# oooolga/Ctrl-V

Hardware: AMD Instinct MI355X
Metric: denoising steps/sec, SVD+ControlNet 25f 576x1024 (higher is better)
Workload: dtype bf16; 1 GPU; box2video: ControlNet + UNet forward, CFG batch 2, 25 frames, latent 72x128, 25-step Karras Euler schedule, random-init SVD-XT weights; clips_per_gpu=1, parallelism=clip-shard x1, hip_graph=True

## Files before the change

### ctrlv_amd/csrc/abi.hip

```cpp
#include <stdarg.h>
#include <stdlib.h>

#include <mutex>

#include "common.h"

#ifndef CTRLV_BUILD_ID
#define CTRLV_BUILD_ID "unstamped"
#endif

static thread_local char g_err[512] = "";
void ctrlv_set_error(const char* fmt, ...) {
  va_list ap;
  va_start(ap, fmt);
  vsnprintf(g_err, sizeof(g_err), fmt, ap);
  va_end(ap);
}

const ctrlv_debug_t& ctrlv_debug() {
  static const ctrlv_debug_t dbg = [] {
    auto env = [](const char* name, int dflt) { const char* e = getenv(name); return e ? atoi(e) : dflt; };
    ctrlv_debug_t d;
    d.w16 = env("CTRLV_W16", 1);
    d.splitk = env("CTRLV_SPLITK", 1);
    d.force_tile = env("CTRLV_GEMM_FORCE_TILE", 0);
    d.conv_halo = env("CTRLV_CONV_HALO", 1);
    d.gn_fused = env("CTRLV_GN_FUSED", 1);
    d.gn_cross = env("CTRLV_GN_CROSS", 1);
    d.gn_rev = env("CTRLV_GN_REV", 1);
    d.gn_rows = env("CTRLV_GN_ROWS", 256);
    if (d.gn_rows < 32 || d.gn_rows > 1024) d.gn_rows = 256;
    d.ln_rows = env("CTRLV_LN_ROWS", 1);
    d.ff_fused = env("CTRLV_FF_FUSED", 1);
    d.ff_ln = env("CTRLV_FF_LN", 0);
    d.pp_balanced = env("CTRLV_PP_BALANCED", 1);
    d.pp_cgrp = env("CTRLV_PP_CGRP", 0);
    d.attn_rows = env("CTRLV_ATTN_ROWS", 0);
    d.temporal_fused = env("CTRLV_TEMPORAL_FUSED", 1);
    d.wgrad_pp = env("CTRLV_WGRAD_PP", 1);
    d.wgrad_slabs = env("CTRLV_WGRAD_SLABS", 0);
    d.up_phase = env("CTRLV_UP_PHASE", 1);
    return d;
  }();
  return dbg;
}

int ctrlv_current_device() {
  int dev = 0;
  if (hipGetDevice(&dev) != hipSuccess || dev < 0 || dev >= CTRLV_MAX_DEVICES) dev = 0;
  return dev;
}

int ctrlv_num_cu(int dev) {
  static int cu[CTRLV_MAX_DEVICES] = {};
  static std::mutex mu;
  std::lock_guard<std::mutex> lk(mu);
  if (cu[dev] == 0) {
    int n = 0;
    if (hipDeviceGetAttribute(&n, hipDeviceAttributeMultiprocessorCount, dev) != hipSuccess || n <= 0) n = 256;
    cu[dev] = n;
  }
  return cu[dev];
}

extern "C" int ctrlv_last_error(char* buf, size_t n) {
  if (buf && n) {
    strncpy(buf, g_err, n - 1);
    buf[n - 1] = 0;
  }
  return (int)strlen(g_err);
}

extern "C" int ctrlv_abi_version(void) { return 22; }
static_assert(sizeof(ctrlv_gemm_desc) == 264 && offsetof(ctrlv_gemm_desc, ld_raw) == 192 && offsetof(ctrlv_gemm_desc, pad_br) == 196 &&
                  offsetof(ctrlv_gemm_desc, raw_out) == 200,
              "ctrlv_gemm_desc layout changed: that is an ABI bump");
extern "C" int ctrlv_elem_dtype(void) { return CTRLV_ELEM_DTYPE; }

extern "C" int ctrlv_build_id(char* buf, size_t n) {
  static const char marker[] = "CTRLV_BUILD_ID=" CTRLV_BUILD_ID;
  const char* id = marker + 15;
  if (buf && n) {
    strncpy(buf, id, n - 1);
    buf[n - 1] = 0;
  }
  return (int)strlen(id);
}
// ... 1 lines not shown
```

### ctrlv_amd/csrc/ff_fused.hip

```cpp
#include <type_traits>

#include "common.h"
#include "gemm_pp_kernel.h"

namespace {

constexpr int kC = 320, kHid = 1280, kChunks = kHid / 16;
constexpr int kTileM = 128;
#ifndef CTRLV_FF_GEA
#define CTRLV_FF_GEA 6
#endif
constexpr int kGeA = CTRLV_FF_GEA;
constexpr int kNQ = 6;
constexpr int kW1Pieces = 21;
constexpr int kW1Slot = kW1Pieces * 1024, kW2Slot = 10 * 1024;
constexpr int kStgOff = 0;
constexpr int kHfOff = kStgOff + 8 * 4096;
constexpr int kW1Off = kHfOff + 16 * 1024;
constexpr int kW2Off = kW1Off + 3 * kW1Slot;
constexpr int kTabOff = kW2Off + 4 * kW2Slot;
constexpr int kSmem = kTabOff + kGeluTabBytes;
static_assert(kSmem <= 160 * 1024, "fused feed-forward tile does not fit the LDS");

struct FfArgs {
  const el_t* x; int ldx;
  const el_t* w1f; const el_t* w2f;
  ctrlv_gemm_desc o;
  const float* vtab; int vdiv, vmod, ldv;
  const float* ln_g; const float* ln_b; float ln_eps;
  const float* lnv; int ln_vdiv, ln_vmod, ln_ldv;
};

template <int EPI, bool LO = false, bool LN = false>
__global__ __launch_bounds__(512) void ff_fused_kernel(const FfArgs a) {
#if defined(__HIP_DEVICE_COMPILE__)
  extern __shared__ __attribute__((aligned(1024))) char smem[];
  const int lane = threadIdx.x & 63;
  const int wid = __builtin_amdgcn_readfirstlane(threadIdx.x >> 6);
  const int rg = wid & 3, hh = wid >> 2;
  const int r32 = lane & 31, hsel = lane >> 5;
  const ctrlv_gemm_desc& d = a.o;
  const int M = d.M;
  const int tiles = (M + kTileM - 1) / kTileM, G = gridDim.x;

  CTRLV_CLOCK_BEGIN();
  gelu_table_fill(smem + kTabOff, threadIdx.x, 512);

  const __amdgpu_buffer_rsrc_t rsW1 = __builtin_amdgcn_make_buffer_rsrc((void*)a.w1f, 0, kChunks * kW1Slot, 0x00020000);
  const __amdgpu_buffer_rsrc_t rsW2 = __builtin_amdgcn_make_buffer_rsrc((void*)a.w2f, 0, kChunks * kW2Slot, 0x00020000);
  const __amdgpu_buffer_rsrc_t rsX = __builtin_amdgcn_make_buffer_rsrc((void*)a.x, 0, (int)((long)d.M * a.ldx * 2), 0x00020000);
  const __amdgpu_buffer_rsrc_t rsB2 = __builtin_amdgcn_make_buffer_rsrc((void*)(d.bias ? d.bias : (const float*)a.w1f), 0,
                                                                         d.bias ? kC * 4 : 0, 0x00020000);
  auto dma_w1 = [&](int chunk, int g) {
    char* s1 = smem + kW1Off + (g % 3) * kW1Slot;
#pragma unroll
    for (int k = 0; k < 6; ++k) {
      const int pi = k * 4 + rg;
      if (pi < kW1Pieces)
        __builtin_amdgcn_raw_ptr_buffer_load_lds(rsW1, LDS_PTR(s1 + pi * 1024), 16, lane * 16, chunk * kW1Slot + pi * 1024, 0, 0);
    }
  };
  auto dma_w2 = [&](int chunk, int g) {
    char* s2 = smem + kW2Off + (g & 3) * kW2Slot;
#pragma unroll
    for (int k = 0; k < 3; ++k) {
      const int pi = k * 4 + rg;
      if (pi < 10)
        __builtin_amdgcn_raw_ptr_buffer_load_lds(rsW2, LDS_PTR(s2 + pi * 1024), 16, lane * 16, chunk * kW2Slot + pi * 1024, 0, 0);
    }
  };
  for (int i = threadIdx.x * 16; i < 4 * kW2Slot; i += 512 * 16) *(uint4*)(smem + kW2Off + i) = make_uint4(0, 0, 0, 0);
  if (hh == 0) dma_w1(0, 0); else dma_w1(1, 1);
  wait_vmcnt<0>();
  __syncthreads();
  const char* tab = smem + kTabOff;
  const unsigned tab_lds = (unsigned)(unsigned long)LDS_PTR(smem + kTabOff);
  char* const hfx = smem + kHfOff + rg * 4096 + lane * 16;
  const unsigned xone1 = hsel == 0 ? (CTRLV_ELEM_DTYPE == 1 ? 0x3C003C00u : 0x3F803F80u) : 0u;

  int gbase = 0;
  elx8 xr[20];
  u32x4_t ini_b, ini_v;
  const __amdgpu_buffer_rsrc_t rsVt = __builtin_amdgcn_make_buffer_rsrc(
      (void*)(a.vtab ? a.vtab : (const float*)a.w1f), 0, a.vtab ? (int)((long)a.vmod * a.ldv * 4) : 0, 0x00020000);
  auto tile_loads = [&](int tile) {
    const int bm = tile * kTileM;
    const unsigned xoff = (unsigned)(bm + rg * 32 + r32) * (unsigned)(a.ldx * 2) + 16 * hsel;
#pragma unroll
    for (int ks = 0; ks < 20; ++ks)
      xr[ks] = __builtin_bit_cast(elx8, __builtin_amdgcn_raw_buffer_load_b128(rsX, xoff, ks * 32, 0));
    const unsigned col4 = lane < 40 ? (unsigned)(hh * 160 + lane * 4) * 4 : 0xFFFFFFFFu;
    ini_b = __builtin_amdgcn_raw_buffer_load_b128(rsB2, col4, 0, 0);
    ini_v = __builtin_amdgcn_raw_buffer_load_b128(rsVt, col4, a.vtab ? ((bm / a.vdiv) % a.vmod) * (a.ldv * 4) : 0, 0);
  };
  tile_loads(blockIdx.x);
  for (int tile = blockIdx.x; tile < tiles; tile += G, gbase += kChunks) {
    const int bm = tile * kTileM;
    const int m = bm + rg * 32 + r32;
#ifdef CTRLV_FF_STAMP
    unsigned long long st_tb; asm volatile("s_memtime %0\n\ts_waitcnt lgkmcnt(0)" : "=s"(st_tb)::"memory");
#endif
    if constexpr (LN) {
      const float* lv = a.lnv ? a.lnv + (long)((m / a.ln_vdiv) % a.ln_vmod) * a.ln_ldv + 8 * hsel : nullptr;
      auto raw8 = [&](int ks, float* f) {
        unpack_elx8(__builtin_bit_cast(uint4, xr[ks]), f);
        if (lv) {
          const float4 p = *(const float4*)(lv + ks * 16), q = *(const float4*)(lv + ks * 16 + 4);
          f[0] += p.x; f[1] += p.y; f[2] += p.z; f[3] += p.w; f[4] += q.x; f[5] += q.y; f[6] += q.z; f[7] += q.w;
        }
      };
      float pilot;
      {
        float f0[8];
        raw8(0, f0);
        pilot = __shfl(f0[0], r32);
      }
      float sm = 0.f, sq = 0.f;
#pragma unroll
      for (int ks = 0; ks < 20; ++ks) {
        float f[8];
        raw8(ks, f);
#pragma unroll
        for (int e = 0; e < 8; ++e) { const float dl = f[e] - pilot; sm += dl; sq += dl * dl; }
        if (ks % 5 == 4) __builtin_amdgcn_sched_barrier(0);
      }
      sm += __shfl_xor(sm, 32);
      sq += __shfl_xor(sq, 32);
      const float dm = sm * (1.0f / kC);
      const float var = sq * (1.0f / kC) - dm * dm;
      const float mean = pilot + dm, rstd = rsqrtf((var > 0.f ? var : 0.f) + a.ln_eps);
      const float* gp = a.ln_g + 8 * hsel;
      const float* bp = a.ln_b + 8 * hsel;
#pragma unroll
      for (int ks = 0; ks < 20; ++ks) {
        float f[8];
        raw8(ks, f);
        const float4 g0 = *(const float4*)(gp + ks * 16), g1 = *(const float4*)(gp + ks * 16 + 4);
        const float4 b0 = *(const float4*)(bp + ks * 16), b1v = *(const float4*)(bp + ks * 16 + 4);
        const float gg[8] = {g0.x, g0.y, g0.z, g0.w, g1.x, g1.y, g1.z, g1.w};
        const float bb[8] = {b0.x, b0.y, b0.z, b0.w, b1v.x, b1v.y, b1v.z, b1v.w};
#pragma unroll
        for (int e = 0; e < 8; ++e) f[e] = (f[e] - mean) * rstd * gg[e] + bb[e];
        uint4 o = pack_elx8(f);
        if (!(m < M)) o = make_uint4(0, 0, 0, 0);
        xr[ks] = __builtin_bit_cast(elx8, o);
        if (ks % 5 == 4) __builtin_amdgcn_sched_barrier(0);
      }
    }
    f32x16 acc[1][5];
    char* const stg = smem + kStgOff + wid * 4096;
    {
      const f32x4 b = __builtin_bit_cast(f32x4, ini_b), w = __builtin_bit_cast(f32x4, ini_v);
      if (lane < 40) *(float4*)(stg + lane * 16) = make_float4(b.x + w.x, b.y + w.y, b.z + w.z, b.w + w.w);
      __builtin_amdgcn_wave_barrier();
#pragma unroll
      for (int i = 0; i < 20; ++i) {
        const int n = i >> 2, q = i & 3;
        const float4 v = *(const float4*)(stg + (n * 32 + 8 * q + 4 * hsel) * 4);
        acc[0][n][4 * q] = v.x; acc[0][n][4 * q + 1] = v.y; acc[0][n][4 * q + 2] = v.z; acc[0][n][4 * q + 3] = v.w;
      }
      asm volatile("s_waitcnt lgkmcnt(0)" ::: "memory");
    }
#ifdef CTRLV_FF_STAMP
#define FSTAMP(v) unsigned long long v; asm volatile("s_memtime %0\n\ts_waitcnt lgkmcnt(0)" : "=s"(v)::"memory")
    unsigned long long st_g1 = 0, st_ge = 0, st_b = 0, st_bar = 0, st_dma = 0, st_tile0;
    { FSTAMP(tt0); st_tile0 = tt0; }
#else
#define FSTAMP(v)
#endif
    elx8 hcur, hprev;
    {
      const uint4 z = make_uint4(0, 0, 0, 0);
      hcur = hprev = __builtin_bit_cast(elx8, z);
    }
    auto geglu_part = [&](auto e0c, auto e1c, const float* av, const float* gv, float* h) {
      constexpr int E0 = decltype(e0c)::value, E1 = decltype(e1c)::value, NE = E1 - E0;
      float fr[NE ? NE : 1];
      f32x2_t te[NE ? NE : 1];
#pragma unroll
      for (int e = 0; e < NE; ++e) {
#pragma clang fp contract(off)
        float tq = __builtin_fmaf(gv[E0 + e], 100.0f, 512.0f);
        tq = __builtin_amdgcn_fmed3f(tq, 0.0f, 1023.99994f);
        fr[e] = __builtin_amdgcn_fractf(tq);
        const unsigned addr = tab_lds + (unsigned)((int)tq) * 8u;
        asm volatile("ds_read_b64 %0, %1" : "=v"(te[e]) : "v"(addr));
      }
      static_assert(NE == 0 || NE == 2 || NE == 4 || NE == 6 || NE == 8, "columns per part");
      if constexpr (NE == 8)
        asm volatile("s_waitcnt lgkmcnt(0)"
                     : "+v"(te[0]), "+v"(te[1]), "+v"(te[2]), "+v"(te[3]), "+v"(te[4]), "+v"(te[5]), "+v"(te[6]), "+v"(te[7]));
      if constexpr (NE == 2) asm volatile("s_waitcnt lgkmcnt(0)" : "+v"(te[0]), "+v"(te[1]));
      if constexpr (NE == 4) asm volatile("s_waitcnt lgkmcnt(0)" : "+v"(te[0]), "+v"(te[1]), "+v"(te[2]), "+v"(te[3]));
      if constexpr (NE == 6)
        asm volatile("s_waitcnt lgkmcnt(0)" : "+v"(te[0]), "+v"(te[1]), "+v"(te[2]), "+v"(te[3]), "+v"(te[4]), "+v"(te[5]));
#pragma unroll
      for (int e = 0; e < NE; ++e) h[E0 + e] = geglu_tab_finish(av[E0 + e], gv[E0 + e], fr[e], make_float2(te[e].x, te[e].y));
    };
    uint32_t hpk[kGeA / 2];
    float ak[kGeA < 8 ? 8 - kGeA : 1], gk[kGeA < 8 ? 8 - kGeA : 1];
    auto seg_g1 = [&](int t) {
      FSTAMP(t0);
      __builtin_amdgcn_s_setprio(2);
      const char* s1 = smem + kW1Off + ((gbase + t) % 3) * kW1Slot + lane * 16;
      elx8 wq[kNQ];
#pragma unroll
      for (int i = 0; i < kNQ; ++i) wq[i] = *(const elx8*)(s1 + i * 1024);
      f32x16 a1;
#pragma unroll
      for (int e = 0; e < 16; ++e) a1[e] = 0.f;
      __builtin_amdgcn_sched_barrier(0);
#pragma unroll
      for (int ks = 0; ks < 21; ++ks) {
        elx8 xf;
        if (ks == 20) {
          unsigned one = xone1;
          asm volatile("" : "+v"(one));
          xf = __builtin_bit_cast(elx8, make_uint4(one, 0, 0, 0));
        } else {
          xf = xr[ks];
        }
        a1 = mfma_32x32x16(wq[ks % kNQ], xf, a1);
        if (ks + kNQ < 21) wq[ks % kNQ] = *(const elx8*)(s1 + (ks + kNQ) * 1024);
        __builtin_amdgcn_sched_barrier(0);
      }
      FSTAMP(t1);
      float av[8], gv[8], h[8];
#pragma unroll
      for (int e = 0; e < 8; ++e) { av[e] = a1[e]; gv[e] = a1[8 + e]; }
      geglu_part(std::integral_constant<int, 0>{}, std::integral_constant<int, kGeA>{}, av, gv, h);
#pragma unroll
      for (int e = 0; e < kGeA / 2; ++e) hpk[e] = pack_elx2(h[2 * e], h[2 * e + 1]);
#pragma unroll
      for (int e = 0; e < 8 - kGeA; ++e) { ak[e] = av[kGeA + e]; gk[e] = gv[kGeA + e]; }
      __builtin_amdgcn_s_setprio(0);
#ifdef CTRLV_FF_STAMP
      FSTAMP(t2);
      st_g1 += t1 - t0; st_ge += t2 - t1;
#endif
    };
    auto seg_ge = [&](int t) {
      FSTAMP(t1b);
      float av[8], gv[8], h[8];
#pragma unroll
      for (int e = 0; e < 8 - kGeA; ++e) { av[kGeA + e] = ak[e]; gv[kGeA + e] = gk[e]; }
      geglu_part(std::integral_constant<int, kGeA>{}, std::integral_constant<int, 8>{}, av, gv, h);
      uint32_t hw[4];
#pragma unroll
      for (int e = 0; e < 4; ++e) hw[e] = e < kGeA / 2 ? hpk[e] : pack_elx2(h[2 * e], h[2 * e + 1]);
      const uint4 hp = make_uint4(hw[0], hw[1], hw[2], hw[3]);
      *(uint4*)(hfx + (t & 3) * 1024) = hp;
      hprev = hcur;
      hcur = __builtin_bit_cast(elx8, hp);
#ifdef CTRLV_FF_STAMP
      FSTAMP(t2);
      st_ge += t2 - t1b;
#endif
    };
    auto seg_dma = [&](int t) {
      FSTAMP(t0);
      dma_w1((t + 2) % kChunks, gbase + t + 2);
      if ((t & 1) == 0) { dma_w2(t, gbase + t); dma_w2(t + 1, gbase + t + 1); }
#ifdef CTRLV_FF_STAMP
      FSTAMP(t1);
      st_dma += t1 - t0;
#endif
    };
    auto seg_b = [&](int j) {
      FSTAMP(t0);
      const int c0 = 2 * j;
      const bool live = j >= 0 && j < kChunks / 2;
      const elx8 hpart = *(const elx8*)(hfx + ((c0 + (hh ^ 1)) & 3) * 1024);
      const char* s2a = smem + kW2Off + ((gbase + c0) & 3) * kW2Slot + (5 * hh) * 1024 + lane * 16;
      const char* s2b = smem + kW2Off + ((gbase + c0 + 1) & 3) * kW2Slot + (5 * hh) * 1024 + lane * 16;
      elx8 vq[6];
#pragma unroll
      for (int i = 0; i < 6; ++i) vq[i] = *(const elx8*)((i < 5 ? s2a + i * 1024 : s2b + (i - 5) * 1024));
      const uint4 hz = make_uint4(0, 0, 0, 0);
      const uint4 hp_u = __builtin_bit_cast(uint4, hpart);
      const uint4 own_u = hh == 0 ? __builtin_bit_cast(uint4, hprev) : __builtin_bit_cast(uint4, hcur);
      const uint4 h0_u = !live ? hz : hh == 0 ? own_u : hp_u;
      const uint4 h1_u = !live ? hz : hh == 0 ? hp_u : own_u;
      const elx8 h0 = __builtin_bit_cast(elx8, h0_u), h1 = __builtin_bit_cast(elx8, h1_u);
      __builtin_amdgcn_sched_barrier(0);
#pragma unroll
      for (int i = 0; i < 10; ++i) {
        acc[0][i % 5] = mfma_32x32x16(vq[i % 6], i < 5 ? h0 : h1, acc[0][i % 5]);
        if (i + 6 < 10) vq[i % 6] = *(const elx8*)(s2b + (i + 6 - 5) * 1024);
        __builtin_amdgcn_sched_barrier(0);
      }
#ifdef CTRLV_FF_STAMP
      FSTAMP(t1);
      st_b += t1 - t0;
#endif
    };
    auto slot_barrier = [&](bool dma_wave) {
      FSTAMP(b0);
      if (dma_wave) wait_vmcnt<0>();
      lds_done_barrier();
#ifdef CTRLV_FF_STAMP
      FSTAMP(b1);
      st_bar += b1 - b0;
#endif
    };
    if (hh == 1) { slot_barrier(true); seg_dma(0); }
    for (int k = 0; k < kChunks / 2; ++k) {
      slot_barrier(false);
      seg_g1(2 * k + hh);
      slot_barrier(true);
      seg_ge(2 * k + hh);
      if (2 * k + 1 + hh < kChunks) seg_dma(2 * k + 1 + hh);
      seg_b(k - 1 + hh);
    }
    tile_loads(tile + G);
    slot_barrier(false);
    if (hh == 0) {
      FSTAMP(b0);
      wait_vmcnt<22>();
      lds_done_barrier();
#ifdef CTRLV_FF_STAMP
      FSTAMP(b1);
      st_bar += b1 - b0;
#endif
    }
    hprev = hcur;
    seg_b(kChunks / 2 - 1 + hh);
#ifdef CTRLV_FF_STAMP
    if (lane == 0 && a.lnv) {
      FSTAMP(tt1);
      unsigned long long* o = (unsigned long long*)a.lnv + ((long)blockIdx.x * 8 + wid) * 8;
      o[0] += st_g1; o[1] += st_ge; o[2] += st_dma; o[3] += st_b; o[4] += st_bar; o[5] += tt1 - st_tile0;
      o[6] += st_tile0 - st_tb;
    }
    unsigned long long st_e0; asm volatile("s_memtime %0\n\ts_waitcnt lgkmcnt(0)" : "=s"(st_e0)::"memory");
#endif
    int lane_e = lane;
    asm volatile("" : "+v"(lane_e));
    gemm_epilogue_lds<1, 5, false, EPI, false, false, LO>(d, acc, bm, 0, rg, hh, 32, 160, lane_e, stg, stg + 1024, stg + 2048,
                                                          stg + 3072, nullptr, tab);
    asm volatile("s_waitcnt lgkmcnt(0)" ::: "memory");
#ifdef CTRLV_FF_STAMP
    if (lane == 0 && a.lnv) {
      asm volatile("s_waitcnt vmcnt(0)" ::: "memory");
      unsigned long long st_e1; asm volatile("s_memtime %0\n\ts_waitcnt lgkmcnt(0)" : "=s"(st_e1)::"memory");
      ((unsigned long long*)a.lnv + ((long)blockIdx.x * 8 + wid) * 8)[7] += st_e1 - st_e0;
    }
#endif
  }
  wait_vmcnt<0>();
  CTRLV_CLOCK_END();
#endif
}

__global__ void ff_pack_kernel(const el_t* __restrict__ w1p, const float* __restrict__ b1, const el_t* __restrict__ w2p,
                               el_t* __restrict__ w1f, el_t* __restrict__ w2f) {
  const long i = (long)blockIdx.x * blockDim.x + threadIdx.x;
  const long n1 = (long)kChunks * kW1Pieces * 64 * 8, n2 = (long)kChunks * 10 * 64 * 8;
  if (i < n1) {
    const int j = i & 7, lane = (i >> 3) & 63;
    const int ks = (int)((i >> 9) % kW1Pieces), chunk = (int)(i / (kW1Pieces * 512));
    el_t v = 0;
    if (ks < 20) {
      v = w1p[(long)(chunk * 32 + (lane & 31)) * kC + ks * 16 + 8 * (lane >> 5) + j];
    } else if (lane < 32 && j < 2) {
      const float b = b1[chunk * 32 + lane];
      const el_t hi = f32_to_el(b);
      v = j == 0 ? hi : f32_to_el(b - el_to_f32(hi));
    }
    w1f[i] = v;
  } else if (i < n1 + n2) {
    const long k = i - n1;
    const int j = k & 7, lane = (k >> 3) & 63;
    const int n = (int)((k >> 9) % 10), chunk = (int)(k / (10 * 512));
    w2f[k] = w2p[(long)(n * 32 + (lane & 31)) * kHid + chunk * 16 + 8 * (j >> 2) + 4 * (lane >> 5) + (j & 3)];
  }
}

template <int EPI, bool LO, bool LN>
int launch_ff_ln(const FfArgs& a, hipStream_t stream) {
  static bool attr_set[CTRLV_MAX_DEVICES] = {};
  auto kfn = ff_fused_kernel<EPI, LO, LN>;
  const int dev = ctrlv_current_device();
  if (!attr_set[dev]) {
    CTRLV_HIP_TRY(hipFuncSetAttribute((const void*)kfn, hipFuncAttributeMaxDynamicSharedMemorySize, kSmem));
    attr_set[dev] = true;
  }
  const int num_cu = ctrlv_num_cu(dev);
  const int tiles = (a.o.M + kTileM - 1) / kTileM;
  int grid = tiles;
  if (tiles > num_cu) {
    const int rounds = (tiles + num_cu - 1) / num_cu;
    grid = (tiles + rounds - 1) / rounds;
  }
  hipLaunchKernelGGL(kfn, dim3(grid), dim3(512), kSmem, stream, a);
  CTRLV_LAUNCH_CHECK();
  return CTRLV_OK;
}

template <int EPI, bool LO = false>
int launch_ff(const FfArgs& a, hipStream_t stream) {
  return a.ln_g ? launch_ff_ln<EPI, LO, true>(a, stream) : launch_ff_ln<EPI, LO, false>(a, stream);
}

}

CTRLV_CLOCK_READER(ff_fused)

extern "C" int ctrlv_ff_fused_w1f_bytes(void) { return kChunks * kW1Slot; }

extern "C" int ctrlv_ff_fused_pack(const void* w1_packed, const float* b1, const void* w2_packed, void* w1f, void* w2f,
                                   ctrlv_stream_t stream) {
  CTRLV_CHECK_ARG(w1_packed && b1 && w2_packed && w1f && w2f, "ctrlv_ff_fused_pack: null pointer");
  const long n = (long)kChunks * (kW1Pieces + 10) * 64 * 8;
  hipLaunchKernelGGL(ff_pack_kernel, dim3((unsigned)((n + 255) / 256)), dim3(256), 0, (hipStream_t)stream,
                     (const el_t*)w1_packed, b1, (const el_t*)w2_packed, (el_t*)w1f, (el_t*)w2f);
  CTRLV_LAUNCH_CHECK();
  return CTRLV_OK;
}

static int ff_check(const ctrlv_gemm_desc& d, int ldx, bool report, bool* fold) {
#define FF_REQ(cond, code, ...)                        \
  do {                                                 \
    if (!(cond)) {                                     \
      if (report) ctrlv_set_error(__VA_ARGS__);        \
      return code;                                     \
    }                                                  \
  } while (0)
  *fold = false;
  FF_REQ(d.out != nullptr, CTRLV_E_BAD_ARG, "ctrlv_ff_fused: null pointer");
  FF_REQ(d.M > 0 && d.N == kC && d.Cin == kHid && d.taps == 1 && d.mode == 0 && ldx >= kC && ldx % 8 == 0, CTRLV_E_BAD_SHAPE,
         "ctrlv_ff_fused: serves M x 320 <- 1280 <- 320 only (N=%d Cin=%d ldx=%d)", d.N, d.Cin, ldx);
  FF_REQ(!d.geglu && !d.act && !d.out_f32 && !d.raw_out && !d.A2 && d.n_scale2 == 0, CTRLV_E_BAD_ARG,
         "ctrlv_ff_fused: plain element-type output only");
  FF_REQ(d.n_store == kC && d.ldo % 8 == 0 && (!d.R1 || d.ldr1 % 8 == 0) && (!d.R2 || d.ldr2 % 8 == 0), CTRLV_E_BAD_SHAPE,
         "ctrlv_ff_fused: n_store must be 320 and the row pitches multiples of 8");
  const long lim = 0xFFFFFFF0L;
  FF_REQ((long)d.M * d.ldo * 2 <= lim && (long)d.M * ldx * 2 <= lim && (!d.R1 || (long)d.M * d.ldr1 * 2 <= lim) &&
             (!d.R2 || (long)d.M * d.ldr2 * 2 <= lim),
         CTRLV_E_BAD_SHAPE, "ctrlv_ff_fused: operands beyond 32-bit byte offsets");
  FF_REQ(!d.R2 || d.R1, CTRLV_E_BAD_ARG, "ctrlv_ff_fused: R2 without R1");
  if (pp_split_io(d)) {
    FF_REQ(CTRLV_ELEM_DTYPE == 1 && d.R1 && (!d.R1_lo || d.R1) && (!d.R2_lo || d.R2), CTRLV_E_BAD_ARG,
           "ctrlv_ff_fused: split trunk planes need the fp16 element library and an R1 operand");
  }
  if (d.vmode) {
    FF_REQ((d.vmode == 1 || d.vmode == 2) && d.V && d.vdiv > 0 && d.vmod > 0 && d.ldv >= kC && d.ldv % 4 == 0 &&
               (d.vmode == 1 || d.vS > 0),
           CTRLV_E_BAD_ARG, "ctrlv_ff_fused: bad row-vector operand");
    *fold = d.vmode == 1 && d.vdiv % 256 == 0 && d.s_acc == 1.0f;
    FF_REQ(*fold || !d.R2, CTRLV_E_BAD_ARG,
           "ctrlv_ff_fused: R1 + R2 + a row vector is served only in the per-tile form (vmode 1, vdiv %% 256 == 0, s_acc 1)");
    FF_REQ(*fold || !pp_split_io(d), CTRLV_E_BAD_ARG, "ctrlv_ff_fused: split trunk planes with a row vector: per-tile form only");
  }
  return CTRLV_OK;
#undef FF_REQ
}

extern "C" int ctrlv_ff_fused_ln(const void* x, int ldx, const float* ln_gamma, const float* ln_beta, float ln_eps,
                                 const float* ln_V, int ln_vdiv, int ln_vmod, int ln_ldv, const void* w1f, const void* w2f,
                                 const ctrlv_gemm_desc* out_desc, ctrlv_stream_t stream) {
  CTRLV_CHECK_ARG(x && w1f && w2f && out_desc && out_desc->out, "ctrlv_ff_fused: null pointer");
  CTRLV_CHECK_ARG((ln_gamma == nullptr) == (ln_beta == nullptr), "ctrlv_ff_fused: LayerNorm needs gamma and beta");
#ifndef CTRLV_FF_STAMP
  CTRLV_CHECK_ARG(!ln_V || (ln_gamma && ln_vdiv > 0 && ln_vmod > 0 && ln_ldv >= 320 && ln_ldv % 4 == 0),
                  "ctrlv_ff_fused: bad LayerNorm row-vector table");
#endif
  FfArgs a;
  a.ln_g = ln_gamma; a.ln_b = ln_beta; a.ln_eps = ln_eps;
  a.lnv = ln_V; a.ln_vdiv = ln_V ? ln_vdiv : 1; a.ln_vmod = ln_V ? ln_vmod : 1; a.ln_ldv = ln_ldv;
  a.x = (const el_t*)x; a.ldx = ldx; a.w1f = (const el_t*)w1f; a.w2f = (const el_t*)w2f;
  a.o = *out_desc;
  a.vtab = nullptr; a.vdiv = 1; a.vmod = 1; a.ldv = 0;
  bool fold = false;
  const int rc = ff_check(a.o, ldx, true, &fold);
  if (rc != CTRLV_OK) return rc;
  if (fold) {
    a.vtab = a.o.V; a.vdiv = a.o.vdiv; a.vmod = a.o.vmod; a.ldv = a.o.ldv;
    a.o.vmode = 0; a.o.V = nullptr;
  }
  const ctrlv_gemm_desc& d = a.o;
  hipStream_t st = (hipStream_t)stream;
#ifdef CTRLV_ELEM_F16
  if (pp_split_io(d)) {
    if (pp_epi_of(d) == 2) return launch_ff<2, true>(a, st);
    if (pp_epi_of(d) == 6) return launch_ff<6, true>(a, st);
  }
#endif
  switch (pp_split_io(d) ? -1 : pp_epi_of(d)) {
    case 0: return launch_ff<0>(a, st);
    case 1: return launch_ff<1>(a, st);
    case 2: return launch_ff<2>(a, st);
    case 3: return launch_ff<3>(a, st);
    case 6: return launch_ff<6>(a, st);
    default: break;
  }
  ctrlv_set_error("ctrlv_ff_fused: epilogue operand combination not served (bias [+ V], + R1 [+ V], + R1 + R2 [+ a per-tile V])");
  return CTRLV_E_BAD_ARG;
}

extern "C" int ctrlv_ff_fused(const void* x, int ldx, const void* w1f, const void* w2f,
                              const ctrlv_gemm_desc* out_desc, ctrlv_stream_t stream) {
  return ctrlv_ff_fused_ln(x, ldx, nullptr, nullptr, 0.f, nullptr, 1, 1, 0, w1f, w2f, out_desc, stream);
}

extern "C" int ctrlv_ff_fused_serves(const ctrlv_gemm_desc* out_desc, int ldx) {
  if (!out_desc) return 0;
  bool fold = false;
  if (ff_check(*out_desc, ldx, false, &fold) != CTRLV_OK) return 0;
  return (out_desc->act || (out_desc->out_f32 & 1)) ? 0 : 1;
}
```

### ctrlv_amd/csrc/plan.hip

```cpp
#include <math.h>

#include <string>
#include <unordered_map>
#include <vector>

#include "common.h"

#define TRY(expr)                   \
  do {                              \
    int rc__ = (expr);              \
    if (rc__ != CTRLV_OK) return rc__; \
  } while (0)

namespace {

__device__ __forceinline__ float ld_any(const void* p, int dtype, long i) {
  if (dtype == 0) return ((const float*)p)[i];
  if (dtype == 1) return (float)((const _Float16*)p)[i];
  return bf16_to_f32(((const bf16_t*)p)[i]);
}
__device__ __forceinline__ int row_map(int n, int N, int geglu) {
  if (!geglu) return n;
  const int inner = N >> 1, isg = n >= inner, r = isg ? n - inner : n;
  return ((r >> 4) * 2 + isg) * 16 + (r & 15);
// ... 597 lines not shown

int frame_embedding(Ctx& c, const Transformer& t, int F, float* e) {
  const int C = t.C, kp = t.tpe1.k;
  const size_t mk = c.mark();
  float* ar = (float*)c.alloc((size_t)F * 4);
  el_t* te = c.rows(F, kp);
  el_t* hh = c.rows(F, 4 * C);
  el_t* tmp = kp != C ? c.rows(F, C) : nullptr;
  if (!c.dry) {
    if (c.overflow) { ctrlv_set_error("plan forward: workspace too small"); return CTRLV_E_BAD_ARG; }
    hipLaunchKernelGGL(arange_kernel, dim3((F + 63) / 64), dim3(64), 0, c.st, ar, F);
    CTRLV_LAUNCH_CHECK();
    if (kp != C) {
      CTRLV_HIP_TRY(hipMemsetAsync(te, 0, (size_t)F * kp * 2, c.st));
      TRY(ctrlv_timestep_embedding(ar, F, C, tmp, c.st));
      CTRLV_HIP_TRY(hipMemcpy2DAsync(te, (size_t)kp * 2, tmp, (size_t)C * 2, (size_t)C * 2, F, hipMemcpyDeviceToDevice, c.st));
    } else {
      TRY(ctrlv_timestep_embedding(ar, F, C, te, c.st));
    }
  }
  {
    ctrlv_gemm_desc d = gd(te, kp, t.tpe1, hh, 4 * C, F, t.tpe1.n, kp, 4 * C);
    d.act = 1;
    TRY(gemm(c, d));
  }
  {
    ctrlv_gemm_desc d = gd(hh, 4 * C, t.tpe2, e, C, F, t.tpe2.n, 4 * C, C);
    d.out_f32 = 1;
    TRY(gemm(c, d));
  }
  c.release(mk);
  return CTRLV_OK;
}

int ff_pair(Ctx& c, const FeedFwd& f, ctrlv_gemm_desc proj, ctrlv_gemm_desc outd, int C, el_t** u) {
  if (ctrlv_debug().ff_fused && f.w1f && ctrlv_ff_fused_serves(&outd, proj.lda)) {
    if (c.dry) return CTRLV_OK;
    if (c.overflow) { ctrlv_set_error("plan forward: workspace too small (need >= %zu bytes)", c.peak); return CTRLV_E_BAD_ARG; }
    ProfScope ps(c, CTRLV_FAM_GEMM_LINEAR, 2.0 * outd.M * 320.0 * (2560 + 1280),
                 (double)outd.M * 320 * (2 * (2 + (outd.R1 ? 1 : 0) + (outd.R2 ? 1 : 0)) + (outd.R1_lo ? 1 : 0) + (outd.R2_lo ? 1 : 0) +
                                         (outd.out_lo ? 1 : 0)), outd.M, 320, 320, 0x100);
    return ctrlv_ff_fused(proj.A, proj.lda, f.w1f, f.w2f, &outd, c.st);
  }
  if (*u == nullptr) *u = c.rows(proj.M, 4 * C);
  proj.out = *u;
  outd.A = *u;
  TRY(gemm(c, proj));
  TRY(gemm(c, outd));
  return CTRLV_OK;
}

int ln_ff(Ctx& c, const FeedFwd& f, const Norm& nm, const Trk& xraw, const float* lnV, int lnvdiv, int lnvmod, int lnldv,
          el_t* tt, const ctrlv_gemm_desc& proj, const ctrlv_gemm_desc& outd, int C, el_t** u) {
  if (ctrlv_debug().ff_fused && ctrlv_debug().ff_ln && f.w1f && !xraw.lo && ctrlv_ff_fused_serves(&outd, C)) {
    if (c.dry) return CTRLV_OK;
    if (c.overflow) { ctrlv_set_error("plan forward: workspace too small (need >= %zu bytes)", c.peak); return CTRLV_E_BAD_ARG; }
    ProfScope ps(c, CTRLV_FAM_GEMM_LINEAR, 2.0 * outd.M * 320.0 * (2560 + 1280),
                 (double)outd.M * 320 * 2 * (2 + (outd.R1 ? 1 : 0) + (outd.R2 ? 1 : 0)), outd.M, 320, 320, 0x300);
    return ctrlv_ff_fused_ln(xraw.hi, C, nm.g, nm.b, 1e-5f, lnV, lnvdiv, lnvmod, lnldv, f.w1f, f.w2f, &outd, c.st);
  }
  TRY(layernorm(c, xraw, proj.M, C, nm, tt, lnV, lnvdiv, lnvmod, lnldv));
  return ff_pair(c, f, proj, outd, C, u);
}

int run_tr(Ctx& c, const Transformer& t, const Trk& x, int H, int W, Trk* out_) {
  const int B = c.B, F = c.F, C = t.C, N = B * F, S = H * W;
  const long M = (long)N * S;
  const Trk out = c.trunk(M, C);
  const size_t mk = c.mark();
  const float* emb = t.frame_emb;
  if (F != c.p->cfg.num_frames || emb == nullptr) {
    float* e = (float*)c.alloc((size_t)F * C * 4);
    TRY(frame_embedding(c, t, F, e));
    emb = e;
  }
  el_t* tt = c.rows(M, C);
  if (c.gn_cross_valid && !c.dry) {
    c.gn_cross_valid = false;
    ProfScope ps(c, CTRLV_FAM_GROUPNORM, 0.0, 2.0 * 2 * N * (double)S * C, N * S, C, 1);
    TRY(ctrlv_groupnorm_from_partials_split(x.hi, x.lo, N, S, C, 1, 1e-6f, c.gn_cross, t.gn.g, t.gn.b, 0, tt, c.st));
  } else {
    TRY(groupnorm(c, x, Trk{}, 0, N, S, C, 1, t.gn, 1e-6f, 0, tt));
  }
  const Trk h0 = c.trunk(M, C);
  {
    ctrlv_gemm_desc d = gd(tt, C, t.pin, h0.hi, C, (int)M, C, C, C);
    set_out(d, h0);
    TRY(gemm(c, d));
  }
  TRY(layernorm(c, h0, (int)M, C, t.s_ln1, tt));
  el_t* qkv = c.rows(M, 3 * C);
  {
    ctrlv_gemm_desc d = gd(tt, C, t.s_qkv, qkv, 3 * C, (int)M, 3 * C, C, 3 * C);
    d.n_scale2 = C; d.s_acc2 = 0.125f * 1.44269504088896340736f;
    TRY(gemm(c, d));
  }
  el_t* a = c.rows(M, C);
  if (!c.dry) {
    ProfScope ps(c, CTRLV_FAM_ATTENTION_SPATIAL, 4.0 * N * (C / 64) * (double)S * S * 64, 2.0 * 4 * N * (double)S * C, N, S, C);
    TRY(ctrlv_attention_spatial_prescaled(qkv, a, N, S, C, c.st));
  }
  const Trk h1 = c.trunk(M, C);
  {
    ctrlv_gemm_desc d = gd(a, C, t.s_o, h1.hi, C, (int)M, C, C, C);
    set_out(d, h1);
    set_r1(d, h0, C);
    d.V = c.xattn + t.xattn_off[0]; d.ldv = c.ldx; d.vmode = 1; d.vdiv = F * S;
    TRY(gemm(c, d));
  }
  el_t* u = nullptr;
  const Trk h2 = h0;
// ... 638 lines not shown
```

### ctrlv_amd/models/blocks.py

```python
import math
import os

import torch
from torch import nn

from .. import ops, packing
from ..lora import merged_weight


class FwdCtx:

    def __init__(self, ws, B, F, temb, xattn, time_context_order):
        self.ws, self.B, self.F = ws, B, F
        self.temb = temb
        self.xattn = xattn
        self.quirk = time_context_order == "sb"
        self.gn_part = None
        self.gn_cross = None
        self.gn_cross_valid = False
        self.trace = None


def _sigmoid(x):
    return 1.0 / (1.0 + math.exp(-x))
# ... 66 lines not shown
        self.norm3 = nn.LayerNorm(dim)
        self.ff = _FeedForward(dim)


class _TemporalBasicTransformerBlock(nn.Module):
    def __init__(self, dim, heads, dim_head, cross_dim):
        super().__init__()
        self.norm_in = nn.LayerNorm(dim)
        self.ff_in = _FeedForward(dim, dim)
        self.norm1 = nn.LayerNorm(dim)
        self.attn1 = _Attention(dim, heads, dim_head)
        self.norm2 = nn.LayerNorm(dim)
        self.attn2 = _Attention(dim, heads, dim_head, cross_dim)
        self.norm3 = nn.LayerNorm(dim)
        self.ff = _FeedForward(dim)


def _f32(t):
    return t.detach().float().contiguous()


def _lo(t):
    return getattr(t, "lo", None) if t is not None else None


def _trk_epi(epi, out):
    e = dict(epi)
    for k in ("R1", "R2"):
        if _lo(e.get(k)) is not None:
            e[k + "_lo"] = _lo(e[k])
    if _lo(out) is not None:
        e["out_lo"] = _lo(out)
    return e


_FF_FUSED = os.environ.get("CTRLV_FF_FUSED", "1") != "0"
_TEMPORAL_FUSED = os.environ.get("CTRLV_TEMPORAL_FUSED", "1") != "0"


def _ff_pair(ws, x, ffp, ubox, out, C, rows_per_image=0, **epi):
    wproj, bproj, wout, bout = ffp[:4]
    epi = _trk_epi(epi, out)
    if _FF_FUSED and len(ffp) == 6 and ops.ff_fused_serves(x, out, **epi):
        ops.ff_fused(x, ffp[4], ffp[5], out, bias=bout, **epi)
        return
    M = x.shape[0]
    if ubox[0] is None:
        ubox[0] = ws.alloc((M, 4 * C))
    u = ubox[0]
    ops.gemm(x, wproj, u, N=8 * C, cin=C, bias=bproj, geglu=1)
    ops.gemm(u, wout, out, N=C, cin=4 * C, bias=bout, rows_per_image=rows_per_image, **epi)


_FF_LN = os.environ.get("CTRLV_FF_LN", "0") not in ("", "0")


def _ln_ff(ws, xraw, ln, t, ffp, ubox, out, C, ln_V=None, ln_vdiv=1, ln_vmod=1 << 30, rows_per_image=0, **epi):
    if _FF_FUSED and _FF_LN and len(ffp) == 6 and _lo(xraw) is None and ops.ff_fused_serves(xraw, out, **_trk_epi(epi, out)):
        ops.ff_fused(xraw, ffp[4], ffp[5], out, bias=ffp[3], ln=(ln[0], ln[1], 1e-5), ln_V=ln_V, ln_vdiv=ln_vdiv,
                     ln_vmod=ln_vmod, **_trk_epi(epi, out))
        return
    if ln_V is not None:
        ops.layernorm(xraw, ln[0], ln[1], 1e-5, t, V=ln_V, vdiv=ln_vdiv, vmod=ln_vmod, x_lo=_lo(xraw))
    else:
        ops.layernorm(xraw, ln[0], ln[1], 1e-5, t, x_lo=_lo(xraw))
    _ff_pair(ws, t, ffp, ubox, out, C, rows_per_image=rows_per_image, **epi)


def _gn_scratch(ctx, n_img, S, C, ips):
    need = ops.groupnorm_scratch_floats(n_img, S, C, ips)
    if ctx.gn_part is None or ctx.gn_part.numel() < need:
        ctx.gn_part = torch.empty(max(need, 1 << 18), dtype=torch.float32, device=ctx.ws.device)
    return ctx.gn_part


def _gemm_groupnorm(ctx, A, W, out, gkw, n_img, S, C, ips, gamma, beta, eps, y):
    gkw = _trk_epi(gkw, out)
    if S % 64 == 0 and ops.gemm_gn_partials_serves(A, W, out, **gkw):
        need = ops.groupnorm_fused_scratch_floats(n_img, S, ips)
        if ctx.gn_part is None or ctx.gn_part.numel() < need:
            ctx.gn_part = torch.empty(max(need, 1 << 18), dtype=torch.float32, device=ctx.ws.device)
        ops.gemm(A, W, out, gn_partials=ctx.gn_part, **gkw)
        ops.groupnorm_from_partials(out, n_img, S, C, ips, gamma, beta, eps, True, y, ctx.gn_part, x_lo=_lo(out))
    else:
        ops.gemm(A, W, out, **gkw)
        ops.groupnorm(out, None, n_img, S, C, ips, gamma, beta, eps, True, y, _gn_scratch(ctx, n_img, S, C, ips),
                      x_lo=_lo(out))


class SpatioTemporalResBlock(nn.Module):
    def __init__(self, in_channels, out_channels, temb_channels, eps=1e-6):
        super().__init__()
        self.cin, self.cout, self.eps = in_channels, out_channels, eps
        self.spatial_res_block = _ResnetBlock2D(in_channels, out_channels, temb_channels, eps)
        self.temporal_res_block = _TemporalResnetBlock(out_channels, temb_channels, eps)
        self.time_mixer = _AlphaBlender(0.5)
        self.temb_off = None
        self._pk = None

    def temb_projections(self):
        return [self.spatial_res_block.time_emb_proj, self.temporal_res_block.time_emb_proj]

    def pack(self):
        s, t = self.spatial_res_block, self.temporal_res_block
        pk = dict(
            g1=_f32(s.norm1.weight), b1=_f32(s.norm1.bias), w1=packing.pack_conv3x3(s.conv1.weight),
            cb1=_f32(s.conv1.bias),
            g2=_f32(s.norm2.weight), b2=_f32(s.norm2.bias), w2=packing.pack_conv3x3(s.conv2.weight),
            cb2=_f32(s.conv2.bias),
            tg1=_f32(t.norm1.weight), tb1=_f32(t.norm1.bias), tw1=packing.pack_conv_temporal(t.conv1.weight),
            tcb1=_f32(t.conv1.bias),
# ... 346 lines not shown
```

Measured before the change: 4.598 steps/s.

## Enable LayerNorm fused into feed-forward kernel with LDS-staged gamma/beta and row vector

Turns on by default the path that folds the LayerNorm into the fused feed-forward kernel, removing a separate layernorm pass and its activation round trip through memory. The in-kernel LayerNorm is rewritten to stage gamma, beta and the per-tile row vector in LDS via buffer-to-LDS DMA, with software-pipelined ds_reads and permlane32 swaps instead of shuffles. To fit LDS, the hidden-fragment staging buffer is halved from four slots to two. A new constraint requires the row vector to be constant across 128-row tiles, otherwise the code falls back to the unfused path.

```diff
diff --git a/ctrlv_amd/csrc/abi.hip b/ctrlv_amd/csrc/abi.hip
--- a/ctrlv_amd/csrc/abi.hip
+++ b/ctrlv_amd/csrc/abi.hip
@@ -32,7 +32,7 @@
     if (d.gn_rows < 32 || d.gn_rows > 1024) d.gn_rows = 256;
     d.ln_rows = env("CTRLV_LN_ROWS", 1);
     d.ff_fused = env("CTRLV_FF_FUSED", 1);
-    d.ff_ln = env("CTRLV_FF_LN", 0);
+    d.ff_ln = env("CTRLV_FF_LN", 1);
     d.pp_balanced = env("CTRLV_PP_BALANCED", 1);
     d.pp_cgrp = env("CTRLV_PP_CGRP", 0);
     d.attn_rows = env("CTRLV_ATTN_ROWS", 0);
diff --git a/ctrlv_amd/csrc/ff_fused.hip b/ctrlv_amd/csrc/ff_fused.hip
--- a/ctrlv_amd/csrc/ff_fused.hip
+++ b/ctrlv_amd/csrc/ff_fused.hip
@@ -16,10 +16,13 @@
 constexpr int kW1Slot = kW1Pieces * 1024, kW2Slot = 10 * 1024;
 constexpr int kStgOff = 0;
 constexpr int kHfOff = kStgOff + 8 * 4096;
-constexpr int kW1Off = kHfOff + 16 * 1024;
+constexpr int kW1Off = kHfOff + 8 * 1024;
 constexpr int kW2Off = kW1Off + 3 * kW1Slot;
 constexpr int kTabOff = kW2Off + 4 * kW2Slot;
-constexpr int kSmem = kTabOff + kGeluTabBytes;
+constexpr int kLnOff = kTabOff + kGeluTabBytes;
+constexpr int kLnVOff = kLnOff + 2 * kC * 4 + 512;
+constexpr int kSmem = kLnVOff + 2048;
+static_assert(kLnVOff % 1024 == 0, "LDS-DMA pieces are 1 KiB aligned here");
 static_assert(kSmem <= 160 * 1024, "fused feed-forward tile does not fit the LDS");
 
 struct FfArgs {
@@ -31,7 +34,115 @@
   const float* lnv; int ln_vdiv, ln_vmod, ln_ldv;
 };
 
-template <int EPI, bool LO = false, bool LN = false>
+template <int K = 0, class F>
+__device__ __forceinline__ void ln_for20(F&& f) {
+  if constexpr (K < 20) {
+    f(std::integral_constant<int, K>{});
+    ln_for20<K + 1>(f);
+  }
+}
+__device__ __forceinline__ void ln_pin(elx8& v) { asm volatile("" : "+v"(v)); }
+template <int OFF>
+__device__ __forceinline__ void ln_read2(f32x4 (&q)[2], unsigned addr) {
+  asm volatile("ds_read_b128 %0, %1 offset:%2" : "=v"(q[0]) : "v"(addr), "n"(OFF) : "memory");
+  asm volatile("ds_read_b128 %0, %1 offset:%2" : "=v"(q[1]) : "v"(addr), "n"(OFF + 16) : "memory");
+}
+template <int N>
+__device__ __forceinline__ void ln_wait2(f32x4 (&q)[2]) {
+  asm volatile("s_waitcnt lgkmcnt(%2)" : "+v"(q[0]), "+v"(q[1]) : "n"(N));
+}
+__device__ __forceinline__ float ln_swap_sum(float v) {
+  auto r = __builtin_amdgcn_permlane32_swap(__float_as_uint(v), __float_as_uint(v), false, false);
+  return __uint_as_float(r[0]) + __uint_as_float(r[1]);
+}
+template <bool HASV>
+__device__ __forceinline__ void ln_fragments(elx8 (&xr)[20], unsigned gb_lds, unsigned v_lds, float eps, bool keep, int hsel) {
+  f32x4 vq[2][2];
+  auto raw8 = [&](int ks, float* f) {
+    ln_pin(xr[ks]);
+    unpack_elx8(__builtin_bit_cast(uint4, xr[ks]), f);
+    if constexpr (HASV) {
+      const f32x4 p = vq[ks & 1][0], q = vq[ks & 1][1];
+      f[0] += p.x; f[1] += p.y; f[2] += p.z; f[3] += p.w; f[4] += q.x; f[5] += q.y; f[6] += q.z; f[7] += q.w;
+    }
+  };
+  auto v_step = [&](auto ksc) {
+    constexpr int ks = decltype(ksc)::value;
+    if constexpr (HASV) {
+      if constexpr (ks + 1 < 20) {
+        ln_read2<(ks + 1) * 64>(vq[(ks + 1) & 1], v_lds);
+        ln_wait2<2>(vq[ks & 1]);
+      } else {
+        ln_wait2<0>(vq[ks & 1]);
+      }
+    }
+  };
+  float pilot;
+  {
+    if constexpr (HASV) { ln_read2<0>(vq[0], v_lds); ln_wait2<0>(vq[0]); }
+    float f0[8];
+    raw8(0, f0);
+    const unsigned own = __float_as_uint(f0[0]);
+    auto r = __builtin_amdgcn_permlane32_swap(own, own, false, false);
+    const unsigned other = r[0] == own ? r[1] : r[0];
+    pilot = __uint_as_float(hsel ? other : own);
+  }
+  float sm = 0.f, sq = 0.f;
+  auto pass1 = [&](auto ksc) {
+    constexpr int ks = decltype(ksc)::value;
+    v_step(ksc);
+    float f[8];
+    raw8(ks, f);
+#pragma unroll
+    for (int e = 0; e < 8; ++e) { const float dl = f[e] - pilot; sm += dl; sq += dl * dl; }
+    __builtin_amdgcn_sched_barrier(0);
+  };
+  auto pass2_all = [&](float mean, float rstd) {
+    f32x4 gq[2][2], bq[2][2];
+    ln_read2<0>(gq[0], gb_lds);
+    ln_read2<kC * 4>(bq[0], gb_lds);
+    if constexpr (HASV) ln_read2<0>(vq[0], v_lds);
+    auto step = [&](auto ksc) {
+      constexpr int ks = decltype(ksc)::value;
+      constexpr int NR = HASV ? 6 : 4;
+      if constexpr (ks + 1 < 20) {
+        ln_read2<(ks + 1) * 64>(gq[(ks + 1) & 1], gb_lds);
+        ln_read2<kC * 4 + (ks + 1) * 64>(bq[(ks + 1) & 1], gb_lds);
+        if constexpr (HASV) ln_read2<(ks + 1) * 64>(vq[(ks + 1) & 1], v_lds);
+        ln_wait2<NR>(gq[ks & 1]);
+        ln_wait2<NR>(bq[ks & 1]);
+        if constexpr (HASV) ln_wait2<NR>(vq[ks & 1]);
+      } else {
+        ln_wait2<0>(gq[ks & 1]);
+        ln_wait2<0>(bq[ks & 1]);
+        if constexpr (HASV) ln_wait2<0>(vq[ks & 1]);
+      }
+      const f32x4 g0 = gq[ks & 1][0], g1 = gq[ks & 1][1], b0 = bq[ks & 1][0], b1 = bq[ks & 1][1];
+      const float gg[8] = {g0.x, g0.y, g0.z, g0.w, g1.x, g1.y, g1.z, g1.w};
+      const float bb[8] = {b0.x, b0.y, b0.z, b0.w, b1.x, b1.y, b1.z, b1.w};
+      float f[8];
+      raw8(ks, f);
+#pragma unroll
+      for (int e = 0; e < 8; ++e) f[e] = (f[e] - mean) * rstd * gg[e] + bb[e];
+      uint4 o = pack_elx8(f);
+      if (!keep) o = make_uint4(0, 0, 0, 0);
+      xr[ks] = __builtin_bit_cast(elx8, o);
+      ln_pin(xr[ks]);
+      __builtin_amdgcn_sched_barrier(0);
+    };
+    ln_for20(step);
+  };
+  ln_for20(pass1);
+  sm = ln_swap_sum(sm);
+  sq = ln_swap_sum(sq);
+  const float dm = sm * (1.0f / kC);
+  const float var = sq * (1.0f / kC) - dm * dm;
+  float mean = pilot + dm, rstd = rsqrtf((var > 0.f ? var : 0.f) + eps);
+  asm volatile("" : "+v"(mean), "+v"(rstd));
+  pass2_all(mean, rstd);
+}
+
+template <int EPI, bool LO = false, int LN = 0>
 __global__ __launch_bounds__(512) void ff_fused_kernel(const FfArgs a) {
 #if defined(__HIP_DEVICE_COMPILE__)
   extern __shared__ __attribute__((aligned(1024))) char smem[];
@@ -45,6 +156,12 @@
 
   CTRLV_CLOCK_BEGIN();
   gelu_table_fill(smem + kTabOff, threadIdx.x, 512);
+  if constexpr (LN) {
+    for (int i = threadIdx.x; i < kC; i += 512) {
+      *(float*)(smem + kLnOff + i * 4) = a.ln_g[i];
+      *(float*)(smem + kLnOff + (kC + i) * 4) = a.ln_b[i];
+    }
+  }
 
   const __amdgpu_buffer_rsrc_t rsW1 = __builtin_amdgcn_make_buffer_rsrc((void*)a.w1f, 0, kChunks * kW1Slot, 0x00020000);
   const __amdgpu_buffer_rsrc_t rsW2 = __builtin_amdgcn_make_buffer_rsrc((void*)a.w2f, 0, kChunks * kW2Slot, 0x00020000);
@@ -75,17 +192,34 @@
   __syncthreads();
   const char* tab = smem + kTabOff;
   const unsigned tab_lds = (unsigned)(unsigned long)LDS_PTR(smem + kTabOff);
-  char* const hfx = smem + kHfOff + rg * 4096 + lane * 16;
+  char* const hfx = smem + kHfOff + rg * 2048 + lane * 16;
   const unsigned xone1 = hsel == 0 ? (CTRLV_ELEM_DTYPE == 1 ? 0x3C003C00u : 0x3F803F80u) : 0u;
 
   int gbase = 0;
   elx8 xr[20];
   u32x4_t ini_b, ini_v;
+  constexpr bool ln_hasv = LN == 2;
+  const __amdgpu_buffer_rsrc_t rsLv = __builtin_amdgcn_make_buffer_rsrc(
+      (void*)(ln_hasv ? a.lnv : (const float*)a.w1f), 0, ln_hasv ? (int)((long)a.ln_vmod * a.ln_ldv * 4) : 0, 0x00020000);
+  auto ln_vec_dma = [&](int tile) {
+    if constexpr (LN) {
+      if (ln_hasv && wid == 0) {
+        const int vrow = (((tile * kTileM) / a.ln_vdiv) % a.ln_vmod) * (a.ln_ldv * 4);
+        int lane_v = lane;
+        asm volatile("" : "+v"(lane_v));
+        __builtin_amdgcn_raw_ptr_buffer_load_lds(rsLv, LDS_PTR(smem + kLnVOff), 16, lane_v * 16, vrow, 0, 0);
+        __builtin_amdgcn_raw_ptr_buffer_load_lds(rsLv, LDS_PTR(smem + kLnVOff + 1024), 16,
+                                                 lane_v < 16 ? 1024 + lane_v * 16 : 0xFFFFFFFFu, vrow, 0, 0);
+      }
+    }
+  };
   const __amdgpu_buffer_rsrc_t rsVt = __builtin_amdgcn_make_buffer_rsrc(
       (void*)(a.vtab ? a.vtab : (const float*)a.w1f), 0, a.vtab ? (int)((long)a.vmod * a.ldv * 4) : 0, 0x00020000);
   auto tile_loads = [&](int tile) {
     const int bm = tile * kTileM;
-    const unsigned xoff = (unsigned)(bm + rg * 32 + r32) * (unsigned)(a.ldx * 2) + 16 * hsel;
+    int lane_x = lane;
+    if constexpr (LN != 0) asm volatile("" : "+v"(lane_x));
+    const unsigned xoff = (unsigned)(bm + rg * 32 + (lane_x & 31)) * (unsigned)(a.ldx * 2) + 16 * (lane_x >> 5);
 #pragma unroll
     for (int ks = 0; ks < 20; ++ks)
       xr[ks] = __builtin_bit_cast(elx8, __builtin_amdgcn_raw_buffer_load_b128(rsX, xoff, ks * 32, 0));
@@ -93,6 +227,10 @@
     ini_b = __builtin_amdgcn_raw_buffer_load_b128(rsB2, col4, 0, 0);
     ini_v = __builtin_amdgcn_raw_buffer_load_b128(rsVt, col4, a.vtab ? ((bm / a.vdiv) % a.vmod) * (a.ldv * 4) : 0, 0);
   };
+  ln_vec_dma(blockIdx.x);
+  if constexpr (LN) {
+    if (ln_hasv) { wait_vmcnt<0>(); __syncthreads(); }
+  }
   tile_loads(blockIdx.x);
   for (int tile = blockIdx.x; tile < tiles; tile += G, gbase += kChunks) {
     const int bm = tile * kTileM;
@@ -100,55 +238,15 @@
 #ifdef CTRLV_FF_STAMP
     unsigned long long st_tb; asm volatile("s_memtime %0\n\ts_waitcnt lgkmcnt(0)" : "=s"(st_tb)::"memory");
 #endif
+    char* const stg = smem + kStgOff + wid * 4096;
     if constexpr (LN) {
-      const float* lv = a.lnv ? a.lnv + (long)((m / a.ln_vdiv) % a.ln_vmod) * a.ln_ldv + 8 * hsel : nullptr;
-      auto raw8 = [&](int ks, float* f) {
-        unpack_elx8(__builtin_bit_cast(uint4, xr[ks]), f);
-        if (lv) {
-          const float4 p = *(const float4*)(lv + ks * 16), q = *(const float4*)(lv + ks * 16 + 4);
-          f[0] += p.x; f[1] += p.y; f[2] += p.z; f[3] += p.w; f[4] += q.x; f[5] += q.y; f[6] += q.z; f[7] += q.w;
-        }
-      };
-      float pilot;
-      {
-        float f0[8];
-        raw8(0, f0);
-        pilot = __shfl(f0[0], r32);
-      }
-      float sm = 0.f, sq = 0.f;
-#pragma unroll
-      for (int ks = 0; ks < 20; ++ks) {
-        float f[8];
-        raw8(ks, f);
-#pragma unroll
-        for (int e = 0; e < 8; ++e) { const float dl = f[e] - pilot; sm += dl; sq += dl * dl; }
-        if (ks % 5 == 4) __builtin_amdgcn_sched_barrier(0);
-      }
-      sm += __shfl_xor(sm, 32);
-      sq += __shfl_xor(sq, 32);
-      const float dm = sm * (1.0f / kC);
-      const float var = sq * (1.0f / kC) - dm * dm;
-      const float mean = pilot + dm, rstd = rsqrtf((var > 0.f ? var : 0.f) + a.ln_eps);
-      const float* gp = a.ln_g + 8 * hsel;
-      const float* bp = a.ln_b + 8 * hsel;
-#pragma unroll
-      for (int ks = 0; ks < 20; ++ks) {
-        float f[8];
-        raw8(ks, f);
-        const float4 g0 = *(const float4*)(gp + ks * 16), g1 = *(const float4*)(gp + ks * 16 + 4);
-        const float4 b0 = *(const float4*)(bp + ks * 16), b1v = *(const float4*)(bp + ks * 16 + 4);
-        const float gg[8] = {g0.x, g0.y, g0.z, g0.w, g1.x, g1.y, g1.z, g1.w};
-        const float bb[8] = {b0.x, b0.y, b0.z, b0.w, b1v.x, b1v.y, b1v.z, b1v.w};
-#pragma unroll
-        for (int e = 0; e < 8; ++e) f[e] = (f[e] - mean) * rstd * gg[e] + bb[e];
-        uint4 o = pack_elx8(f);
-        if (!(m < M)) o = make_uint4(0, 0, 0, 0);
-        xr[ks] = __builtin_bit_cast(elx8, o);
-        if (ks % 5 == 4) __builtin_amdgcn_sched_barrier(0);
-      }
+      int hs = hsel;
+      asm volatile("" : "+v"(hs));
+      const unsigned gb_lds = (unsigned)(unsigned long)LDS_PTR(smem + kLnOff) + 32u * hs;
+      const unsigned v_lds = (unsigned)(unsigned long)LDS_PTR(smem + kLnVOff) + 32u * hs;
+      ln_fragments<ln_hasv>(xr, gb_lds, v_lds, a.ln_eps, m < M, hs);
     }
     f32x16 acc[1][5];
-    char* const stg = smem + kStgOff + wid * 4096;
     {
       const f32x4 b = __builtin_bit_cast(f32x4, ini_b), w = __builtin_bit_cast(f32x4, ini_v);
       if (lane < 40) *(float4*)(stg + lane * 16) = make_float4(b.x + w.x, b.y + w.y, b.z + w.z, b.w + w.w);
@@ -249,7 +347,7 @@
 #pragma unroll
       for (int e = 0; e < 4; ++e) hw[e] = e < kGeA / 2 ? hpk[e] : pack_elx2(h[2 * e], h[2 * e + 1]);
       const uint4 hp = make_uint4(hw[0], hw[1], hw[2], hw[3]);
-      *(uint4*)(hfx + (t & 3) * 1024) = hp;
+      *(uint4*)(hfx + (t & 1) * 1024) = hp;
       hprev = hcur;
       hcur = __builtin_bit_cast(elx8, hp);
 #ifdef CTRLV_FF_STAMP
@@ -270,7 +368,7 @@
       FSTAMP(t0);
       const int c0 = 2 * j;
       const bool live = j >= 0 && j < kChunks / 2;
-      const elx8 hpart = *(const elx8*)(hfx + ((c0 + (hh ^ 1)) & 3) * 1024);
+      const elx8 hpart = *(const elx8*)(hfx + (hh ^ 1) * 1024);
       const char* s2a = smem + kW2Off + ((gbase + c0) & 3) * kW2Slot + (5 * hh) * 1024 + lane * 16;
       const char* s2b = smem + kW2Off + ((gbase + c0 + 1) & 3) * kW2Slot + (5 * hh) * 1024 + lane * 16;
       elx8 vq[6];
@@ -312,6 +410,7 @@
       if (2 * k + 1 + hh < kChunks) seg_dma(2 * k + 1 + hh);
       seg_b(k - 1 + hh);
     }
+    ln_vec_dma(tile + G);
     tile_loads(tile + G);
     slot_barrier(false);
     if (hh == 0) {
@@ -376,7 +475,7 @@
   }
 }
 
-template <int EPI, bool LO, bool LN>
+template <int EPI, bool LO, int LN>
 int launch_ff_ln(const FfArgs& a, hipStream_t stream) {
   static bool attr_set[CTRLV_MAX_DEVICES] = {};
   auto kfn = ff_fused_kernel<EPI, LO, LN>;
@@ -399,7 +498,12 @@
 
 template <int EPI, bool LO = false>
 int launch_ff(const FfArgs& a, hipStream_t stream) {
-  return a.ln_g ? launch_ff_ln<EPI, LO, true>(a, stream) : launch_ff_ln<EPI, LO, false>(a, stream);
+#ifdef CTRLV_FF_STAMP
+  return a.ln_g ? launch_ff_ln<EPI, LO, 1>(a, stream) : launch_ff_ln<EPI, LO, 0>(a, stream);
+#else
+  return a.ln_g ? (a.lnv ? launch_ff_ln<EPI, LO, 2>(a, stream) : launch_ff_ln<EPI, LO, 1>(a, stream))
+                : launch_ff_ln<EPI, LO, 0>(a, stream);
+#endif
 }
 
 }
@@ -464,6 +568,7 @@
 #ifndef CTRLV_FF_STAMP
   CTRLV_CHECK_ARG(!ln_V || (ln_gamma && ln_vdiv > 0 && ln_vmod > 0 && ln_ldv >= 320 && ln_ldv % 4 == 0),
                   "ctrlv_ff_fused: bad LayerNorm row-vector table");
+  CTRLV_CHECK_ARG(!ln_V || ln_vdiv % kTileM == 0, "ctrlv_ff_fused: the LayerNorm row vector must be constant over 128-row tiles");
 #endif
   FfArgs a;
   a.ln_g = ln_gamma; a.ln_b = ln_beta; a.ln_eps = ln_eps;
diff --git a/ctrlv_amd/csrc/plan.hip b/ctrlv_amd/csrc/plan.hip
--- a/ctrlv_amd/csrc/plan.hip
+++ b/ctrlv_amd/csrc/plan.hip
@@ -673,11 +673,13 @@
 
 int ln_ff(Ctx& c, const FeedFwd& f, const Norm& nm, const Trk& xraw, const float* lnV, int lnvdiv, int lnvmod, int lnldv,
           el_t* tt, const ctrlv_gemm_desc& proj, const ctrlv_gemm_desc& outd, int C, el_t** u) {
-  if (ctrlv_debug().ff_fused && ctrlv_debug().ff_ln && f.w1f && !xraw.lo && ctrlv_ff_fused_serves(&outd, C)) {
+  if (ctrlv_debug().ff_fused && ctrlv_debug().ff_ln && f.w1f && !xraw.lo && (!lnV || lnvdiv % 128 == 0) &&
+      ctrlv_ff_fused_serves(&outd, C)) {
     if (c.dry) return CTRLV_OK;
     if (c.overflow) { ctrlv_set_error("plan forward: workspace too small (need >= %zu bytes)", c.peak); return CTRLV_E_BAD_ARG; }
     ProfScope ps(c, CTRLV_FAM_GEMM_LINEAR, 2.0 * outd.M * 320.0 * (2560 + 1280),
-                 (double)outd.M * 320 * 2 * (2 + (outd.R1 ? 1 : 0) + (outd.R2 ? 1 : 0)), outd.M, 320, 320, 0x300);
+                 (double)outd.M * 320 * (2 * (2 + (outd.R1 ? 1 : 0) + (outd.R2 ? 1 : 0)) + (outd.R1_lo ? 1 : 0) + (outd.R2_lo ? 1 : 0) +
+                                         (outd.out_lo ? 1 : 0)), outd.M, 320, 320, 0x300);
     return ctrlv_ff_fused_ln(xraw.hi, C, nm.g, nm.b, 1e-5f, lnV, lnvdiv, lnvmod, lnldv, f.w1f, f.w2f, &outd, c.st);
   }
   TRY(layernorm(c, xraw, proj.M, C, nm, tt, lnV, lnvdiv, lnvmod, lnldv));
diff --git a/ctrlv_amd/models/blocks.py b/ctrlv_amd/models/blocks.py
--- a/ctrlv_amd/models/blocks.py
+++ b/ctrlv_amd/models/blocks.py
@@ -142,11 +142,12 @@
     ops.gemm(u, wout, out, N=C, cin=4 * C, bias=bout, rows_per_image=rows_per_image, **epi)
 
 
-_FF_LN = os.environ.get("CTRLV_FF_LN", "0") not in ("", "0")
+_FF_LN = os.environ.get("CTRLV_FF_LN", "1") not in ("", "0")
 
 
 def _ln_ff(ws, xraw, ln, t, ffp, ubox, out, C, ln_V=None, ln_vdiv=1, ln_vmod=1 << 30, rows_per_image=0, **epi):
-    if _FF_FUSED and _FF_LN and len(ffp) == 6 and _lo(xraw) is None and ops.ff_fused_serves(xraw, out, **_trk_epi(epi, out)):
+    if (_FF_FUSED and _FF_LN and len(ffp) == 6 and _lo(xraw) is None and (ln_V is None or ln_vdiv % 128 == 0) and
+            ops.ff_fused_serves(xraw, out, **_trk_epi(epi, out))):
         ops.ff_fused(xraw, ffp[4], ffp[5], out, bias=ffp[3], ln=(ln[0], ln[1], 1e-5), ln_V=ln_V, ln_vdiv=ln_vdiv,
                      ln_vmod=ln_vmod, **_trk_epi(epi, out))
         return
```

Result: no change. 4.622 steps/s (median of 6 runs) (+0.5%).
